# Kingsford-Group/squid

Measured on NVIDIA B200. Metric: read pairs/s through segment-graph build, higher is better.
Workload: dtype int32

## Files before the change

### squid_b200/csrc/sq_phase1.cuh

```cuda
#ifndef SQ_PHASE1_CUH
#define SQ_PHASE1_CUH
#include "sq_classify.cuh"
#include "sq_depth_cover.cuh"
#include "sq_stream.cuh"

namespace sq {

struct TileAgg {
    uint64_t okmax;
    uint32_t n_pc, n_dp;
};
struct P1Out {
    uint8_t *cls;
    uint16_t *first_len;
    TileAgg *agg;
    uint32_t *cov_nq; uint64_t *cov_qmax;
    uint64_t *qstage_key; int32_t *qstage_end;
    int32_t *ccmax;
    uint64_t *gate_word;
    int32_t *cand_rec; uint64_t *cand_key; int32_t *n_cand; int32_t cand_cap;
    int32_t *lmax;
    long long *first_kept;
    int32_t *bad_flags;
    int32_t *ticket;
    int32_t n_tiles;
    const struct BatchDesc *desc;
};

constexpr uint32_t kP1Fields = F_REF | F_POS | F_MREF | F_MPOS | F_FLAG | F_TLEN | F_LOWQ | F_MAPQ | F_AUX | F_BLOCKS;

struct BatchDesc { DevBatch b; Params p; };
__device__ __noinline__ ClassifyOut classify_from_hbm(const BatchDesc *desc, int64_t r, int64_t prev) { return classify_record(desc->b, desc->p, r, prev); }

__device__ __forceinline__ void push_candidates(const P1Out &o, unsigned mask, int64_t rec, uint64_t key, int32_t *s_bad) {
    const int lane = threadIdx.x & 31;
    int32_t base = 0;
    if (lane == 0) base = atomicAdd(o.n_cand, __popc(mask));
    base = __shfl_sync(0xffffffffu, base, 0);
    if (mask & (1u << lane)) {
        const int32_t k = base + __popc(mask & ((1u << lane) - 1u));
        if (k < o.cand_cap) { o.cand_rec[k] = (int32_t)rec; o.cand_key[k] = key; }
        else atomicOr(s_bad, 16);
    }
}

__global__ void __launch_bounds__(kTileThreads, 8) k_classify_tiles(DevBatch b, Params p, P1Out o, int bulk_ok) {
    extern __shared__ __align__(128) unsigned char smem_raw[];
    TileStage &s = *reinterpret_cast<TileStage *>(smem_raw);
    __shared__ int s_tile;
    __shared__ uint32_t s_gate[kTileChunks];
    __shared__ int32_t s_cmax[kTileChunks];
    __shared__ int32_t s_pc[kWarpsPerTile], s_dp[kWarpsPerTile], s_qcnt[kTileChunks];
    __shared__ long long s_prev_carry;
    __shared__ int32_t s_bad, s_lmax, s_minkeep, s_ccmax, s_nq, s_qmax;
    int32_t *s_end = s.end_pos;
    uint16_t *s_flen = s.total_len;
    const int tid = threadIdx.x, lane = tid & 31, warp = tid >> 5;
    const unsigned full = 0xffffffffu;
    if (tid == 0) { s_tile = atomicAdd(o.ticket, 1); s_bad = 0; s_lmax = 0; s_minkeep = kTile; s_ccmax = kNoCcEnd; s_nq = 0; s_qmax = -1; }
    __syncthreads();
    const int tile = s_tile;
    const StageTicket tk = stage_issue<kP1Fields>(s, b, nullptr, tile, bulk_ok != 0);
    const TileInfo ti = tk.ti;
    const int n = ti.n;
    const int64_t rec0 = ti.rec0;
    long long walk = -2;
    if (warp == 0) {
        const int64_t q = rec0 - 1 - lane;
        const bool g = q >= 0 && record_gate(b.flag[q], b.mapq[q], b.aux[q], b.ref_id[q], p.min_mapq);
        const unsigned m = __ballot_sync(full, g);
        if (m) walk = rec0 - 1 - (__ffs(m) - 1);
        else if (rec0 <= 32) walk = -1;
    }
    stage_wait<kP1Fields>(s, b, nullptr, tk);
    const TileBatch tb = tile_view(s, ti, b);

#pragma unroll 1
    for (int j = 0; j < kTileRPT; j++) {
        const int i = j * kTileThreads + tid;
        bool g = false;
        int bad = 0;
        if (i < n) {
            const int32_t rid = s.ref_id[i];
            const uint16_t f = s.flag[i];
            g = record_gate(f, s.mapq[i], s.aux[i], rid, p.min_mapq);
            if (rid >= p.n_ref || rid < -1) bad |= 1;
            if (rid < 0 && flag_mapped(f)) bad |= 2;
            const uint32_t o0 = s.blk_off[i], o1 = s.blk_off[i + 1];
            if (o1 < o0 || o1 - o0 > (uint32_t)kMaxBlocks) bad |= 4;
            const int64_t r = rec0 + i;
            if (r + 1 < b.n_rec) {
                const int32_t rid2 = i + 1 < n ? s.ref_id[i + 1] : b.ref_id[r + 1], pos2 = i + 1 < n ? s.pos[i + 1] : b.pos[r + 1];
                const uint64_t k1 = rid < 0 ? ~0ull : (((uint64_t)(uint32_t)rid << 32) | (uint32_t)s.pos[i]);
                const uint64_t k2 = rid2 < 0 ? ~0ull : (((uint64_t)(uint32_t)rid2 << 32) | (uint32_t)pos2);
                if (k2 < k1) bad |= 8;
            }
        }
        const unsigned gm = __ballot_sync(full, g);
        if (lane == 0) s_gate[j * kWarpsPerTile + warp] = gm;
        if (bad) atomicOr(&s_bad, bad);
    }
    __syncthreads();
    const bool usable = !(s_bad & 5);
    const bool staged = ti.nb >= 0;
    if (warp == 0) {
        const uint32_t w = lane < kTileChunks ? s_gate[lane] : 0u;
        const unsigned nz = __ballot_sync(full, w != 0u);
        uint64_t agg = 0;
        if (nz) {
            const int hw = 31 - __clz(nz);
            const uint32_t hv = __shfl_sync(full, w, hw);
            agg = (uint64_t)(rec0 + hw * 32 + (31 - __clz(hv))) + 1ull;
        }
        if (lane == 0) word_publish(o.gate_word, tile, nz ? 2u : 1u, agg);
        if (nz && walk == -2) walk = (long long)word_lookback_max(o.gate_word, tile) - 1;
        if (lane == 0) s_prev_carry = walk;
    }
    __syncthreads();

    const int32_t chr_tile = s.ref_id[0];
    const bool single_chr = chr_tile >= 0 && s.ref_id[n - 1] == chr_tile;
    int32_t flen_max = 0, npc = 0, ndp = 0, cc_max = kNoCcEnd, nq = 0, q_max = -1;
#pragma unroll 1
    for (int j = 0; j < kTileRPT; j++) {
        const int i = j * kTileThreads + tid;
        uint8_t c = 0;
        int32_t key_end = 0, co_len = 0;
        if (i < n && usable && ((s_gate[i >> 5] >> (i & 31)) & 1u)) {
            int word = i >> 5;
            uint32_t m = s_gate[word] & ((1u << (i & 31)) - 1u);
            while (m == 0u && word > 0) { word--; m = s_gate[word]; }
            const int64_t prev = m ? rec0 + word * 32 + (31 - __clz(m)) : (int64_t)s_prev_carry;
            const int64_t r = rec0 + i;
            const ClassifyOut co = (staged && prev >= rec0) ? classify_record(tb, p, r, prev) : classify_from_hbm(o.desc, r, prev);
            c = co.cls; key_end = (int32_t)(uint32_t)co.other_key;
            co_len = co.first_len;
            if (co.first_len > flen_max) flen_max = co.first_len;
            if (co.cc_end > cc_max) cc_max = co.cc_end;
        }
        int32_t qs = -1;
        if (i < n && (c & CLS_GATE)) {
            const uint16_t f = s.flag[i];
            const int32_t rid = s.ref_id[i], ps = s.pos[i], mr = s.mate_ref_id[i], mp = s.mate_pos[i];
            if (cover_qualifies(c, f, rid, ps, mr, mp)) { qs = cover_start(f, rid, ps, mr, mp); if (qs < 0) qs = 0; }
        }
        const int chunk = j * kWarpsPerTile + warp;
        { const int32_t cq = __popc(__ballot_sync(full, qs >= 0)); nq += cq; if (lane == 0) s_qcnt[chunk] = cq; }
        { const int32_t m = __reduce_max_sync(full, qs); if (m > q_max) q_max = m; }
        if (i < n) { s.cls[i] = c; s_end[i] = key_end; s_flen[i] = (uint16_t)(co_len < 65535 ? co_len : 65535); }
        npc += __popc(__ballot_sync(full, (c & CLS_PART) != 0));
        ndp += __popc(__ballot_sync(full, (c & (CLS_CONC | CLS_DISPL)) == (CLS_CONC | CLS_DISPL)));
        const unsigned km = __ballot_sync(full, (c & CLS_KEEP) != 0);
        const int32_t cm = __reduce_max_sync(full, key_end);
        if (lane == 0) { s_cmax[chunk] = cm; if (km) atomicMin(&s_minkeep, chunk * 32 + __ffs(km) - 1); }
    }
    flen_max = __reduce_max_sync(full, flen_max);
    cc_max = __reduce_max_sync(full, cc_max);
    if (lane == 0) { s_pc[warp] = npc; s_dp[warp] = ndp; if (flen_max > 0) atomicMax(&s_lmax, flen_max); if (cc_max > kNoCcEnd) atomicMax(&s_ccmax, cc_max);
                     if (nq) atomicAdd(&s_nq, nq); if (q_max >= 0) atomicMax(&s_qmax, q_max); }
    __syncthreads();
    if (warp == 0) {
        int32_t inc = lane < kTileChunks ? s_cmax[lane] : 0;
#pragma unroll
        for (int d = 1; d < 32; d <<= 1) { const int32_t u = __shfl_up_sync(full, inc, d); if (lane >= d && u > inc) inc = u; }
        const int32_t tot = __shfl_sync(full, inc, 31);
        int32_t exc = __shfl_up_sync(full, inc, 1);
        if (lane == 0) exc = 0;
        if (lane < kTileChunks) s_cmax[lane] = exc;
        if (lane == 0) {
            int32_t a = 0, c2 = 0;
#pragma unroll
            for (int k = 0; k < kWarpsPerTile; k++) { a += s_pc[k]; c2 += s_dp[k]; }
            TileAgg g; g.n_pc = (uint32_t)a; g.n_dp = (uint32_t)c2;
            g.okmax = (single_chr && tot > 0) ? (((uint64_t)(uint32_t)(chr_tile + 1) << 32) | (uint32_t)tot) : 0ull;
            if (single_chr) o.agg[tile] = g;
            else { s_pc[0] = a; s_dp[0] = c2; }
        }
    }
    __syncthreads();
    if (single_chr) {
#pragma unroll 1
        for (int j = 0; j < kTileRPT; j++) {
            const int i = j * kTileThreads + tid, chunk = j * kWarpsPerTile + warp;
            const bool keep = i < n && (s.cls[i] & CLS_KEEP);
            const int32_t pos = i < n ? s.pos[i] : 0;
            const int32_t base = s_cmax[chunk];
            const bool maybe = keep && (base == 0 ? (chr_tile != 0 || pos > p.read_len) : pos > base + p.read_len);
            if (!__any_sync(full, maybe)) continue;
            int32_t v = i < n ? s_end[i] : 0;
#pragma unroll
            for (int d = 1; d < 32; d <<= 1) { const int32_t u = __shfl_up_sync(full, v, d); if (lane >= d && u > v) v = u; }
            int32_t e = __shfl_up_sync(full, v, 1);
            if (lane == 0 || e < base) e = base;
            const bool gap = keep && (e == 0 ? (chr_tile != 0 || pos > p.read_len) : pos > e + p.read_len);
            const unsigned gm = __ballot_sync(full, gap);
            if (gm) push_candidates(o, gm, rec0 + i, e == 0 ? 0ull : (((uint64_t)(uint32_t)(chr_tile + 1) << 32) | (uint32_t)e), &s_bad);
        }
    } else if (tid == 0) {
        uint64_t run = 0;
        for (int i = 0; i < n; i++) {
            if (s.cls[i] & CLS_KEEP) {
                const uint64_t e = run < (1ull << 32) ? (1ull << 32) : run;
                const int32_t oc = (int32_t)(e >> 32) - 1, orr = (int32_t)(uint32_t)e;
                if (s.ref_id[i] != oc || s.pos[i] > orr + p.read_len) {
                    const int32_t k = atomicAdd(o.n_cand, 1);
                    if (k < o.cand_cap) { o.cand_rec[k] = (int32_t)(rec0 + i); o.cand_key[k] = run; }
                    else atomicOr(&s_bad, 16);
                }
            }
            if (s_end[i] != 0) {
                const uint64_t k = ((uint64_t)(uint32_t)(s.ref_id[i] + 1) << 32) | (uint32_t)s_end[i];
                if (k > run) run = k;
            }
        }
        TileAgg g; g.okmax = run; g.n_pc = (uint32_t)s_pc[0]; g.n_dp = (uint32_t)s_dp[0];
        o.agg[tile] = g;
    }
    if (4 * tid + 3 < n) {
        *reinterpret_cast<uint32_t *>(o.cls + rec0 + 4 * tid) = *reinterpret_cast<const uint32_t *>(&s.cls[4 * tid]);
        *reinterpret_cast<uint2 *>(o.first_len + rec0 + 4 * tid) = *reinterpret_cast<const uint2 *>(&s_flen[4 * tid]);
    } else for (int i = 4 * tid; i < n; i++) { o.cls[rec0 + i] = s.cls[i]; o.first_len[rec0 + i] = s_flen[i]; }
    {
        const int32_t cq = lane < kTileChunks ? s_qcnt[lane] : 0;
        int32_t inc = cq;
#pragma unroll
        for (int d = 1; d < 32; d <<= 1) { const int32_t u = __shfl_up_sync(full, inc, d); if (lane >= d) inc += u; }
        const int32_t exc = inc - cq;
#pragma unroll 1
        for (int j = 0; j < kTileRPT; j++) {
            const int i = j * kTileThreads + tid;
            bool q = false;
            uint64_t key = 0;
            if (i < n) {
                const uint8_t c = s.cls[i];
                const uint16_t f = s.flag[i];
                const int32_t rid = s.ref_id[i], ps = s.pos[i], mr = s.mate_ref_id[i], mp = s.mate_pos[i];
                q = cover_qualifies(c, f, rid, ps, mr, mp);
                if (q) key = chrpos_key(rid, cover_start(f, rid, ps, mr, mp));
            }
            const unsigned qm = __ballot_sync(full, q);
            const int32_t before = __shfl_sync(full, exc, j * kWarpsPerTile + warp);
            if (q) {
                const int64_t at = (int64_t)tile * kTile + before + __popc(qm & ((1u << lane) - 1u));
                o.qstage_key[at] = key; o.qstage_end[at] = b.end_pos[rec0 + i];
            }
        }
    }
    __syncthreads();
    if (tid == 0) {
        o.cov_nq[tile] = (uint32_t)s_nq;
        uint64_t qk = 0;
        if (single_chr) { if (s_qmax >= 0) qk = chrpos_key(chr_tile, s_qmax); }
        else for (int i = 0; i < n; i++)
            if ((s.cls[i] & CLS_GATE) && cover_qualifies(s.cls[i], s.flag[i], s.ref_id[i], s.pos[i], s.mate_ref_id[i], s.mate_pos[i])) {
                const uint64_t k = chrpos_key(s.ref_id[i], cover_start(s.flag[i], s.ref_id[i], s.pos[i], s.mate_ref_id[i], s.mate_pos[i]));
                if (k > qk) qk = k;
            }
        o.cov_qmax[tile] = qk;
        o.ccmax[tile] = single_chr ? s_ccmax : kCcWalkTile;
        if (s_lmax > 0) atomicMax(o.lmax, s_lmax);
        if (s_minkeep < kTile) atomicMin(o.first_kept, (long long)(rec0 + s_minkeep));
        if (s_bad) atomicOr(o.bad_flags, s_bad);
    }
}

__global__ void __launch_bounds__(1024) k_tile_scan(TileAgg *agg, int32_t n_tiles, int32_t *totals, uint64_t *ok_total) {
    __shared__ uint64_t s_ok[32];
    __shared__ uint32_t s_pc[32], s_dp[32];
    const int lane = threadIdx.x & 31, warp = threadIdx.x >> 5;
    const unsigned full = 0xffffffffu;
    const int per = ((n_tiles + 31) / 32 + 31) / 32 * 32;
    const int lo = warp * per < n_tiles ? warp * per : n_tiles, hi = (warp + 1) * per < n_tiles ? (warp + 1) * per : n_tiles;
    uint64_t ok = 0; uint32_t pc = 0, dp = 0;
    for (int t = lo + lane; t < hi; t += 32) { const TileAgg g = agg[t]; if (g.okmax > ok) ok = g.okmax; pc += g.n_pc; dp += g.n_dp; }
    ok = warp_max_u64(ok); pc = __reduce_add_sync(full, pc); dp = __reduce_add_sync(full, dp);
    if (lane == 0) { s_ok[warp] = ok; s_pc[warp] = pc; s_dp[warp] = dp; }
    __syncthreads();
    ok = 0; pc = 0; dp = 0;
    for (int w = 0; w < warp; w++) { if (s_ok[w] > ok) ok = s_ok[w]; pc += s_pc[w]; dp += s_dp[w]; }
    if (threadIdx.x == 1023) { totals[1] = (int32_t)(pc + s_pc[31]); totals[2] = (int32_t)(dp + s_dp[31]); }
    for (int base = lo; base < hi; base += 32) {
        const int t = base + lane;
        TileAgg g; g.okmax = 0; g.n_pc = 0; g.n_dp = 0;
        if (t < hi) g = agg[t];
        uint64_t iok = g.okmax; uint32_t ipc = g.n_pc, idp = g.n_dp;
#pragma unroll
        for (int d = 1; d < 32; d <<= 1) {
            const uint64_t a = __shfl_up_sync(full, iok, d);
            const uint32_t x = __shfl_up_sync(full, ipc, d), y = __shfl_up_sync(full, idp, d);
            if (lane >= d) { if (a > iok) iok = a; ipc += x; idp += y; }
        }
        uint64_t eok = __shfl_up_sync(full, iok, 1); uint32_t epc = __shfl_up_sync(full, ipc, 1), edp = __shfl_up_sync(full, idp, 1);
        if (lane == 0) { eok = 0; epc = 0; edp = 0; }
        if (t < hi) { TileAgg e; e.okmax = eok > ok ? eok : ok; e.n_pc = pc + epc; e.n_dp = dp + edp; agg[t] = e; }
        const uint64_t tok = __shfl_sync(full, iok, 31);
        if (tok > ok) ok = tok;
        pc += __shfl_sync(full, ipc, 31); dp += __shfl_sync(full, idp, 31);
    }
    if (threadIdx.x == 1023 && ok_total) *ok_total = ok;
}

__global__ void k_finish_gaps(DevBatch b, const TileAgg *excl, int32_t *cand_rec, uint64_t *cand_key, int32_t n_cand, int32_t read_len, int32_t *totals) {
    const int32_t k = blockIdx.x * blockDim.x + threadIdx.x;
    bool gap = false;
    if (k < n_cand) {
        const int32_t r = cand_rec[k];
        uint64_t e = cand_key[k];
        const uint64_t c = excl[r / kTile].okmax;
        if (c > e) e = c;
        if (e < (1ull << 32)) e = 1ull << 32;
        const int32_t oc = (int32_t)(e >> 32) - 1, orr = (int32_t)(uint32_t)e;
        gap = b.ref_id[r] != oc || b.pos[r] > orr + read_len;
        cand_key[k] = e;
        if (!gap) cand_rec[k] = 0x7fffffff;
    }
    const unsigned m = __ballot_sync(0xffffffffu, gap);
    if ((threadIdx.x & 31) == 0 && m) atomicAdd(&totals[0], __popc(m));
}

__global__ void __launch_bounds__(kTileThreads) k_compact_lists(const uint8_t *cls, int64_t n_rec, const TileAgg *excl, int32_t *pc_rec, int32_t *dp_rec) {
    __shared__ int32_t s_pc[kWarpsPerTile], s_dp[kWarpsPerTile];
    const int tid = threadIdx.x, lane = tid & 31, warp = tid >> 5;
    const int64_t tile = blockIdx.x, rec0 = tile * (int64_t)kTile;
    const int64_t r0 = rec0 + 4 * tid;
    uint32_t w = 0;
    if (r0 + 3 < n_rec) w = *reinterpret_cast<const uint32_t *>(cls + r0);
    else for (int k = 0; k < 4; k++) if (r0 + k < n_rec) w |= (uint32_t)cls[r0 + k] << (8 * k);
    int32_t mypc = 0, mydp = 0;
#pragma unroll
    for (int k = 0; k < 4; k++) {
        const uint32_t c = (w >> (8 * k)) & 0xffu;
        mypc += (c & CLS_PART) ? 1 : 0;
        mydp += ((c & (CLS_CONC | CLS_DISPL)) == (CLS_CONC | CLS_DISPL)) ? 1 : 0;
    }
    if (!__syncthreads_or(mypc | mydp)) return;
    int32_t ipc = mypc, idp = mydp;
#pragma unroll
    for (int d = 1; d < 32; d <<= 1) {
        const int32_t a = __shfl_up_sync(0xffffffffu, ipc, d), c = __shfl_up_sync(0xffffffffu, idp, d);
        if (lane >= d) { ipc += a; idp += c; }
    }
    if (lane == 31) { s_pc[warp] = ipc; s_dp[warp] = idp; }
    __syncthreads();
    int32_t bpc = (int32_t)excl[tile].n_pc, bdp = (int32_t)excl[tile].n_dp;
    for (int k = 0; k < warp; k++) { bpc += s_pc[k]; bdp += s_dp[k]; }
    bpc += ipc - mypc; bdp += idp - mydp;
#pragma unroll
    for (int k = 0; k < 4; k++) {
        const uint32_t c = (w >> (8 * k)) & 0xffu;
        if (c & CLS_PART) pc_rec[bpc++] = (int32_t)(r0 + k);
        if ((c & (CLS_CONC | CLS_DISPL)) == (CLS_CONC | CLS_DISPL)) dp_rec[bdp++] = (int32_t)(r0 + k);
    }
}

}
#endif
```

Before: 2.325 billion.

## Restructure classify tile kernel to warp-contiguous chunks with fewer block barriers

Each warp now owns a contiguous range of 32-record chunks instead of striding across the tile. That lets a warp carry the previous-gated record forward locally, with no backward search over gate words. Per-chunk statistics (qualify masks, keep masks, maxima, counts) go into shared arrays and are reduced once by thread 0, replacing shared atomics, the separate prefix-scan pass and two block barriers. The next-tile boundary record and end_pos loads are prefetched early, and tile_view is rebased to local indices. The cost is more serial work in thread 0 and per-warp serial prefix loops over earlier chunks.

```diff
diff --git a/squid_b200/csrc/sq_phase1.cuh b/squid_b200/csrc/sq_phase1.cuh
--- a/squid_b200/csrc/sq_phase1.cuh
+++ b/squid_b200/csrc/sq_phase1.cuh
@@ -32,7 +32,7 @@
 struct BatchDesc { DevBatch b; Params p; };
 __device__ __noinline__ ClassifyOut classify_from_hbm(const BatchDesc *desc, int64_t r, int64_t prev) { return classify_record(desc->b, desc->p, r, prev); }
 
-__device__ __forceinline__ void push_candidates(const P1Out &o, unsigned mask, int64_t rec, uint64_t key, int32_t *s_bad) {
+__device__ __forceinline__ void push_candidates(const P1Out &o, unsigned mask, int64_t rec, uint64_t key) {
     const int lane = threadIdx.x & 31;
     int32_t base = 0;
     if (lane == 0) base = atomicAdd(o.n_cand, __popc(mask));
@@ -40,7 +40,7 @@
     if (mask & (1u << lane)) {
         const int32_t k = base + __popc(mask & ((1u << lane) - 1u));
         if (k < o.cand_cap) { o.cand_rec[k] = (int32_t)rec; o.cand_key[k] = key; }
-        else atomicOr(s_bad, 16);
+        else atomicOr(o.bad_flags, 16);
     }
 }
 
@@ -48,38 +48,36 @@
     extern __shared__ __align__(128) unsigned char smem_raw[];
     TileStage &s = *reinterpret_cast<TileStage *>(smem_raw);
     __shared__ int s_tile;
-    __shared__ uint32_t s_gate[kTileChunks];
-    __shared__ int32_t s_cmax[kTileChunks];
-    __shared__ int32_t s_pc[kWarpsPerTile], s_dp[kWarpsPerTile], s_qcnt[kTileChunks];
-    __shared__ long long s_prev_carry;
-    __shared__ int32_t s_bad, s_lmax, s_minkeep, s_ccmax, s_nq, s_qmax;
+    __shared__ uint32_t s_gate[kTileChunks], s_kept[kTileChunks], s_qual[kTileChunks];
+    __shared__ int32_t s_cmax[kTileChunks], s_qmax[kTileChunks], s_flmax[kTileChunks], s_ccmax[kTileChunks], s_pc[kTileChunks], s_dp[kTileChunks];
+    __shared__ long long s_walk;
+    __shared__ int32_t s_bad;
     int32_t *s_end = s.end_pos;
     uint16_t *s_flen = s.total_len;
     const int tid = threadIdx.x, lane = tid & 31, warp = tid >> 5;
-    const unsigned full = 0xffffffffu;
-    if (tid == 0) { s_tile = atomicAdd(o.ticket, 1); s_bad = 0; s_lmax = 0; s_minkeep = kTile; s_ccmax = kNoCcEnd; s_nq = 0; s_qmax = -1; }
+    const unsigned full = 0xffffffffu, below = (1u << lane) - 1u;
+    if (tid == 0) { s_tile = atomicAdd(o.ticket, 1); s_bad = 0; }
     __syncthreads();
     const int tile = s_tile;
     const StageTicket tk = stage_issue<kP1Fields>(s, b, nullptr, tile, bulk_ok != 0);
     const TileInfo ti = tk.ti;
     const int n = ti.n;
     const int64_t rec0 = ti.rec0;
-    long long walk = -2;
     if (warp == 0) {
         const int64_t q = rec0 - 1 - lane;
         const bool g = q >= 0 && record_gate(b.flag[q], b.mapq[q], b.aux[q], b.ref_id[q], p.min_mapq);
         const unsigned m = __ballot_sync(full, g);
-        if (m) walk = rec0 - 1 - (__ffs(m) - 1);
-        else if (rec0 <= 32) walk = -1;
-    }
+        if (lane == 0) s_walk = m ? rec0 - 1 - (__ffs(m) - 1) : rec0 <= 32 ? -1 : -2;
+    }
+    int32_t rid_next = -1, pos_next = 0;
+    if (tid == (n - 1) / (kTileRPT * 32) * 32 + ((n - 1) & 31) && rec0 + n < b.n_rec) { rid_next = b.ref_id[rec0 + n]; pos_next = b.pos[rec0 + n]; }
     stage_wait<kP1Fields>(s, b, nullptr, tk);
-    const TileBatch tb = tile_view(s, ti, b);
-
+
+    int bad = 0;
 #pragma unroll 1
-    for (int j = 0; j < kTileRPT; j++) {
-        const int i = j * kTileThreads + tid;
+    for (int k = 0; k < kTileRPT; k++) {
+        const int chunk = warp * kTileRPT + k, i = chunk * 32 + lane;
         bool g = false;
-        int bad = 0;
         if (i < n) {
             const int32_t rid = s.ref_id[i];
             const uint16_t f = s.flag[i];
@@ -90,16 +88,17 @@
             if (o1 < o0 || o1 - o0 > (uint32_t)kMaxBlocks) bad |= 4;
             const int64_t r = rec0 + i;
             if (r + 1 < b.n_rec) {
-                const int32_t rid2 = i + 1 < n ? s.ref_id[i + 1] : b.ref_id[r + 1], pos2 = i + 1 < n ? s.pos[i + 1] : b.pos[r + 1];
+                const int32_t rid2 = i + 1 < n ? s.ref_id[i + 1] : rid_next, pos2 = i + 1 < n ? s.pos[i + 1] : pos_next;
                 const uint64_t k1 = rid < 0 ? ~0ull : (((uint64_t)(uint32_t)rid << 32) | (uint32_t)s.pos[i]);
                 const uint64_t k2 = rid2 < 0 ? ~0ull : (((uint64_t)(uint32_t)rid2 << 32) | (uint32_t)pos2);
                 if (k2 < k1) bad |= 8;
             }
         }
         const unsigned gm = __ballot_sync(full, g);
-        if (lane == 0) s_gate[j * kWarpsPerTile + warp] = gm;
-        if (bad) atomicOr(&s_bad, bad);
-    }
+        if (lane == 0) s_gate[chunk] = gm;
+    }
+    bad = __reduce_or_sync(full, bad);
+    if (lane == 0 && bad) atomicOr(&s_bad, bad);
     __syncthreads();
     const bool usable = !(s_bad & 5);
     const bool staged = ti.nb >= 0;
@@ -109,157 +108,147 @@
         uint64_t agg = 0;
         if (nz) {
             const int hw = 31 - __clz(nz);
-            const uint32_t hv = __shfl_sync(full, w, hw);
-            agg = (uint64_t)(rec0 + hw * 32 + (31 - __clz(hv))) + 1ull;
+            agg = (uint64_t)(rec0 + hw * 32 + (31 - __clz(__shfl_sync(full, w, hw)))) + 1ull;
         }
         if (lane == 0) word_publish(o.gate_word, tile, nz ? 2u : 1u, agg);
-        if (nz && walk == -2) walk = (long long)word_lookback_max(o.gate_word, tile) - 1;
-        if (lane == 0) s_prev_carry = walk;
-    }
-    __syncthreads();
-
-    const int32_t chr_tile = s.ref_id[0];
-    const bool single_chr = chr_tile >= 0 && s.ref_id[n - 1] == chr_tile;
-    int32_t flen_max = 0, npc = 0, ndp = 0, cc_max = kNoCcEnd, nq = 0, q_max = -1;
+    }
+    int32_t last;
+    {
+        const uint32_t w = lane < warp * kTileRPT ? s_gate[lane] : 0u;
+        const unsigned nz = __ballot_sync(full, w != 0u);
+        if (nz) {
+            const int hw = 31 - __clz(nz);
+            last = hw * 32 + (31 - __clz(__shfl_sync(full, w, hw)));
+        } else {
+            long long g = s_walk;
+            const uint32_t own = lane < kTileRPT ? s_gate[warp * kTileRPT + lane] : 0u;
+            if (g == -2 && __any_sync(full, own != 0u)) g = (long long)word_lookback_max(o.gate_word, tile) - 1;
+            last = (int32_t)(g - rec0);
+        }
+    }
+
+    TileInfo tl = ti;
+    tl.rec0 = 0;
+    const TileBatch tb = tile_view(s, tl, b);
 #pragma unroll 1
-    for (int j = 0; j < kTileRPT; j++) {
-        const int i = j * kTileThreads + tid;
+    for (int k = 0; k < kTileRPT; k++) {
+        const int chunk = warp * kTileRPT + k, i = chunk * 32 + lane;
+        const uint32_t gm = usable ? s_gate[chunk] : 0u;
         uint8_t c = 0;
-        int32_t key_end = 0, co_len = 0;
-        if (i < n && usable && ((s_gate[i >> 5] >> (i & 31)) & 1u)) {
-            int word = i >> 5;
-            uint32_t m = s_gate[word] & ((1u << (i & 31)) - 1u);
-            while (m == 0u && word > 0) { word--; m = s_gate[word]; }
-            const int64_t prev = m ? rec0 + word * 32 + (31 - __clz(m)) : (int64_t)s_prev_carry;
-            const int64_t r = rec0 + i;
-            const ClassifyOut co = (staged && prev >= rec0) ? classify_record(tb, p, r, prev) : classify_from_hbm(o.desc, r, prev);
+        int32_t key_end = 0, co_len = 0, cc_end = kNoCcEnd;
+        if ((gm >> lane) & 1u) {
+            const uint32_t m = gm & below;
+            const int32_t prev = m ? chunk * 32 + (31 - __clz(m)) : last;
+            const ClassifyOut co = (staged && prev >= 0) ? classify_record(tb, p, i, prev) : classify_from_hbm(o.desc, rec0 + i, rec0 + prev);
             c = co.cls; key_end = (int32_t)(uint32_t)co.other_key;
-            co_len = co.first_len;
-            if (co.first_len > flen_max) flen_max = co.first_len;
-            if (co.cc_end > cc_max) cc_max = co.cc_end;
-        }
+            co_len = co.first_len; cc_end = co.cc_end;
+        }
+        if (gm) last = chunk * 32 + (31 - __clz(gm));
         int32_t qs = -1;
-        if (i < n && (c & CLS_GATE)) {
+        if (c & CLS_GATE) {
             const uint16_t f = s.flag[i];
             const int32_t rid = s.ref_id[i], ps = s.pos[i], mr = s.mate_ref_id[i], mp = s.mate_pos[i];
             if (cover_qualifies(c, f, rid, ps, mr, mp)) { qs = cover_start(f, rid, ps, mr, mp); if (qs < 0) qs = 0; }
         }
-        const int chunk = j * kWarpsPerTile + warp;
-        { const int32_t cq = __popc(__ballot_sync(full, qs >= 0)); nq += cq; if (lane == 0) s_qcnt[chunk] = cq; }
-        { const int32_t m = __reduce_max_sync(full, qs); if (m > q_max) q_max = m; }
         if (i < n) { s.cls[i] = c; s_end[i] = key_end; s_flen[i] = (uint16_t)(co_len < 65535 ? co_len : 65535); }
-        npc += __popc(__ballot_sync(full, (c & CLS_PART) != 0));
-        ndp += __popc(__ballot_sync(full, (c & (CLS_CONC | CLS_DISPL)) == (CLS_CONC | CLS_DISPL)));
-        const unsigned km = __ballot_sync(full, (c & CLS_KEEP) != 0);
-        const int32_t cm = __reduce_max_sync(full, key_end);
-        if (lane == 0) { s_cmax[chunk] = cm; if (km) atomicMin(&s_minkeep, chunk * 32 + __ffs(km) - 1); }
-    }
-    flen_max = __reduce_max_sync(full, flen_max);
-    cc_max = __reduce_max_sync(full, cc_max);
-    if (lane == 0) { s_pc[warp] = npc; s_dp[warp] = ndp; if (flen_max > 0) atomicMax(&s_lmax, flen_max); if (cc_max > kNoCcEnd) atomicMax(&s_ccmax, cc_max);
-                     if (nq) atomicAdd(&s_nq, nq); if (q_max >= 0) atomicMax(&s_qmax, q_max); }
-    __syncthreads();
-    if (warp == 0) {
-        int32_t inc = lane < kTileChunks ? s_cmax[lane] : 0;
-#pragma unroll
-        for (int d = 1; d < 32; d <<= 1) { const int32_t u = __shfl_up_sync(full, inc, d); if (lane >= d && u > inc) inc = u; }
-        const int32_t tot = __shfl_sync(full, inc, 31);
-        int32_t exc = __shfl_up_sync(full, inc, 1);
-        if (lane == 0) exc = 0;
-        if (lane < kTileChunks) s_cmax[lane] = exc;
-        if (lane == 0) {
-            int32_t a = 0, c2 = 0;
-#pragma unroll
-            for (int k = 0; k < kWarpsPerTile; k++) { a += s_pc[k]; c2 += s_dp[k]; }
-            TileAgg g; g.n_pc = (uint32_t)a; g.n_dp = (uint32_t)c2;
-            g.okmax = (single_chr && tot > 0) ? (((uint64_t)(uint32_t)(chr_tile + 1) << 32) | (uint32_t)tot) : 0ull;
-            if (single_chr) o.agg[tile] = g;
-            else { s_pc[0] = a; s_dp[0] = c2; }
-        }
-    }
-    __syncthreads();
-    if (single_chr) {
-#pragma unroll 1
-        for (int j = 0; j < kTileRPT; j++) {
-            const int i = j * kTileThreads + tid, chunk = j * kWarpsPerTile + warp;
-            const bool keep = i < n && (s.cls[i] & CLS_KEEP);
-            const int32_t pos = i < n ? s.pos[i] : 0;
-            const int32_t base = s_cmax[chunk];
-            const bool maybe = keep && (base == 0 ? (chr_tile != 0 || pos > p.read_len) : pos > base + p.read_len);
-            if (!__any_sync(full, maybe)) continue;
-            int32_t v = i < n ? s_end[i] : 0;
-#pragma unroll
-            for (int d = 1; d < 32; d <<= 1) { const int32_t u = __shfl_up_sync(full, v, d); if (lane >= d && u > v) v = u; }
-            int32_t e = __shfl_up_sync(full, v, 1);
-            if (lane == 0 || e < base) e = base;
-            const bool gap = keep && (e == 0 ? (chr_tile != 0 || pos > p.read_len) : pos > e + p.read_len);
-            const unsigned gm = __ballot_sync(full, gap);
-            if (gm) push_candidates(o, gm, rec0 + i, e == 0 ? 0ull : (((uint64_t)(uint32_t)(chr_tile + 1) << 32) | (uint32_t)e), &s_bad);
-        }
-    } else if (tid == 0) {
-        uint64_t run = 0;
-        for (int i = 0; i < n; i++) {
-            if (s.cls[i] & CLS_KEEP) {
-                const uint64_t e = run < (1ull << 32) ? (1ull << 32) : run;
-                const int32_t oc = (int32_t)(e >> 32) - 1, orr = (int32_t)(uint32_t)e;
-                if (s.ref_id[i] != oc || s.pos[i] > orr + p.read_len) {
-                    const int32_t k = atomicAdd(o.n_cand, 1);
-                    if (k < o.cand_cap) { o.cand_rec[k] = (int32_t)(rec0 + i); o.cand_key[k] = run; }
-                    else atomicOr(&s_bad, 16);
-                }
-            }
-            if (s_end[i] != 0) {
-                const uint64_t k = ((uint64_t)(uint32_t)(s.ref_id[i] + 1) << 32) | (uint32_t)s_end[i];
-                if (k > run) run = k;
-            }
-        }
-        TileAgg g; g.okmax = run; g.n_pc = (uint32_t)s_pc[0]; g.n_dp = (uint32_t)s_dp[0];
-        o.agg[tile] = g;
+        const unsigned qm = __ballot_sync(full, qs >= 0), km = __ballot_sync(full, (c & CLS_KEEP) != 0);
+        const int32_t mq = __reduce_max_sync(full, qs), cm = __reduce_max_sync(full, key_end);
+        const int32_t fm = __reduce_max_sync(full, co_len), ccm = __reduce_max_sync(full, cc_end);
+        const int32_t pc = __popc(__ballot_sync(full, (c & CLS_PART) != 0));
+        const int32_t dp = __popc(__ballot_sync(full, (c & (CLS_CONC | CLS_DISPL)) == (CLS_CONC | CLS_DISPL)));
+        if (lane == 0) { s_qual[chunk] = qm; s_kept[chunk] = km; s_qmax[chunk] = mq; s_cmax[chunk] = cm; s_flmax[chunk] = fm; s_ccmax[chunk] = ccm;
+                         s_pc[chunk] = pc; s_dp[chunk] = dp; }
+    }
+    __syncwarp();
+    int32_t q_end[kTileRPT];
+#pragma unroll
+    for (int k = 0; k < kTileRPT; k++) {
+        const int chunk = warp * kTileRPT + k, i = chunk * 32 + lane;
+        q_end[k] = ((s_qual[chunk] >> lane) & 1u) ? b.end_pos[rec0 + i] : 0;
     }
     if (4 * tid + 3 < n) {
         *reinterpret_cast<uint32_t *>(o.cls + rec0 + 4 * tid) = *reinterpret_cast<const uint32_t *>(&s.cls[4 * tid]);
         *reinterpret_cast<uint2 *>(o.first_len + rec0 + 4 * tid) = *reinterpret_cast<const uint2 *>(&s_flen[4 * tid]);
     } else for (int i = 4 * tid; i < n; i++) { o.cls[rec0 + i] = s.cls[i]; o.first_len[rec0 + i] = s_flen[i]; }
-    {
-        const int32_t cq = lane < kTileChunks ? s_qcnt[lane] : 0;
-        int32_t inc = cq;
-#pragma unroll
-        for (int d = 1; d < 32; d <<= 1) { const int32_t u = __shfl_up_sync(full, inc, d); if (lane >= d) inc += u; }
-        const int32_t exc = inc - cq;
-#pragma unroll 1
-        for (int j = 0; j < kTileRPT; j++) {
-            const int i = j * kTileThreads + tid;
-            bool q = false;
-            uint64_t key = 0;
-            if (i < n) {
-                const uint8_t c = s.cls[i];
-                const uint16_t f = s.flag[i];
-                const int32_t rid = s.ref_id[i], ps = s.pos[i], mr = s.mate_ref_id[i], mp = s.mate_pos[i];
-                q = cover_qualifies(c, f, rid, ps, mr, mp);
-                if (q) key = chrpos_key(rid, cover_start(f, rid, ps, mr, mp));
+    __syncthreads();
+
+    const int32_t chr_tile = s.ref_id[0];
+    const bool single_chr = chr_tile >= 0 && s.ref_id[n - 1] == chr_tile;
+    int32_t run = 0, qat = 0;
+    for (int c = 0; c < warp * kTileRPT; c++) { if (s_cmax[c] > run) run = s_cmax[c]; qat += __popc(s_qual[c]); }
+    int64_t qbase = (int64_t)tile * kTile + qat;
+#pragma unroll
+    for (int k = 0; k < kTileRPT; k++) {
+        const int chunk = warp * kTileRPT + k, i = chunk * 32 + lane;
+        if (single_chr) {
+            const bool keep = i < n && (s.cls[i] & CLS_KEEP);
+            const int32_t pos = i < n ? s.pos[i] : 0;
+            if (__any_sync(full, keep && (run == 0 ? (chr_tile != 0 || pos > p.read_len) : pos > run + p.read_len))) {
+                int32_t v = i < n ? s_end[i] : 0;
+#pragma unroll
+                for (int d = 1; d < 32; d <<= 1) { const int32_t u = __shfl_up_sync(full, v, d); if (lane >= d && u > v) v = u; }
+                int32_t e = __shfl_up_sync(full, v, 1);
+                if (lane == 0 || e < run) e = run;
+                const bool gap = keep && (e == 0 ? (chr_tile != 0 || pos > p.read_len) : pos > e + p.read_len);
+                const unsigned gm = __ballot_sync(full, gap);
+                if (gm) push_candidates(o, gm, rec0 + i, e == 0 ? 0ull : (((uint64_t)(uint32_t)(chr_tile + 1) << 32) | (uint32_t)e));
             }
-            const unsigned qm = __ballot_sync(full, q);
-            const int32_t before = __shfl_sync(full, exc, j * kWarpsPerTile + warp);
-            if (q) {
-                const int64_t at = (int64_t)tile * kTile + before + __popc(qm & ((1u << lane) - 1u));
-                o.qstage_key[at] = key; o.qstage_end[at] = b.end_pos[rec0 + i];
+            if (s_cmax[chunk] > run) run = s_cmax[chunk];
+        }
+        const uint32_t qm = s_qual[chunk];
+        if ((qm >> lane) & 1u) {
+            const uint16_t f = s.flag[i];
+            const int32_t rid = s.ref_id[i], ps = s.pos[i], mr = s.mate_ref_id[i], mp = s.mate_pos[i];
+            const int64_t at = qbase + __popc(qm & below);
+            o.qstage_key[at] = chrpos_key(rid, cover_start(f, rid, ps, mr, mp)); o.qstage_end[at] = q_end[k];
+        }
+        qbase += __popc(qm);
+    }
+
+    if (tid == 0) {
+        int32_t a = 0, c2 = 0, nqt = 0, qmax = -1, tot = 0, lmax = 0, ccm = kNoCcEnd, keep0 = kTile;
+        for (int c = kTileChunks - 1; c >= 0; c--) {
+            a += s_pc[c]; c2 += s_dp[c]; nqt += __popc(s_qual[c]);
+            if (s_qmax[c] > qmax) qmax = s_qmax[c];
+            if (s_cmax[c] > tot) tot = s_cmax[c];
+            if (s_flmax[c] > lmax) lmax = s_flmax[c];
+            if (s_ccmax[c] > ccm) ccm = s_ccmax[c];
+            if (s_kept[c]) keep0 = c * 32 + __ffs(s_kept[c]) - 1;
+        }
+        TileAgg g; g.n_pc = (uint32_t)a; g.n_dp = (uint32_t)c2;
+        uint64_t qk = 0;
+        if (single_chr) {
+            g.okmax = tot > 0 ? (((uint64_t)(uint32_t)(chr_tile + 1) << 32) | (uint32_t)tot) : 0ull;
+            if (qmax >= 0) qk = chrpos_key(chr_tile, qmax);
+        } else {
+            uint64_t okr = 0;
+            for (int i = 0; i < n; i++) {
+                if (s.cls[i] & CLS_KEEP) {
+                    const uint64_t e = okr < (1ull << 32) ? (1ull << 32) : okr;
+                    const int32_t oc = (int32_t)(e >> 32) - 1, orr = (int32_t)(uint32_t)e;
+                    if (s.ref_id[i] != oc || s.pos[i] > orr + p.read_len) {
+                        const int32_t k = atomicAdd(o.n_cand, 1);
+                        if (k < o.cand_cap) { o.cand_rec[k] = (int32_t)(rec0 + i); o.cand_key[k] = okr; }
+                        else atomicOr(o.bad_flags, 16);
+                    }
+                }
+                if (s_end[i] != 0) {
+                    const uint64_t k = ((uint64_t)(uint32_t)(s.ref_id[i] + 1) << 32) | (uint32_t)s_end[i];
+                    if (k > okr) okr = k;
+                }
+                if ((s.cls[i] & CLS_GATE) && cover_qualifies(s.cls[i], s.flag[i], s.ref_id[i], s.pos[i], s.mate_ref_id[i], s.mate_pos[i])) {
+                    const uint64_t k = chrpos_key(s.ref_id[i], cover_start(s.flag[i], s.ref_id[i], s.pos[i], s.mate_ref_id[i], s.mate_pos[i]));
+                    if (k > qk) qk = k;
+                }
             }
-        }
-    }
-    __syncthreads();
-    if (tid == 0) {
-        o.cov_nq[tile] = (uint32_t)s_nq;
-        uint64_t qk = 0;
-        if (single_chr) { if (s_qmax >= 0) qk = chrpos_key(chr_tile, s_qmax); }
-        else for (int i = 0; i < n; i++)
-            if ((s.cls[i] & CLS_GATE) && cover_qualifies(s.cls[i], s.flag[i], s.ref_id[i], s.pos[i], s.mate_ref_id[i], s.mate_pos[i])) {
-                const uint64_t k = chrpos_key(s.ref_id[i], cover_start(s.flag[i], s.ref_id[i], s.pos[i], s.mate_ref_id[i], s.mate_pos[i]));
-                if (k > qk) qk = k;
-            }
+            g.okmax = okr;
+        }
+        o.agg[tile] = g;
+        o.cov_nq[tile] = (uint32_t)nqt;
         o.cov_qmax[tile] = qk;
-        o.ccmax[tile] = single_chr ? s_ccmax : kCcWalkTile;
-        if (s_lmax > 0) atomicMax(o.lmax, s_lmax);
-        if (s_minkeep < kTile) atomicMin(o.first_kept, (long long)(rec0 + s_minkeep));
+        o.ccmax[tile] = single_chr ? ccm : kCcWalkTile;
+        if (lmax > 0) atomicMax(o.lmax, lmax);
+        if (keep0 < kTile) atomicMin(o.first_kept, (long long)(rec0 + keep0));
         if (s_bad) atomicOr(o.bad_flags, s_bad);
     }
 }
```

Result: no change. 2.345 billion, median of 6 (+0.9%).
